# pigBond/olympics-mujoco

Hardware: AMD Instinct MI355X
Metric: env-steps/sec, 4096 UnitreeH1.walk envs per GPU, obs+reward+done+ctrl HIP kernel (higher is better)
Workload: dtype f64; 1 GPU; UnitreeH1.walk config-2: fused K1+K5 over one [T,N] block per step; T=400, envs_per_gpu=4096, launch_regime=[T,N] block per launch, io=qpos/qvel f64 + action f32 in; obs/reward/ctrl f32 + absorbing u8 out, parallelism=env-sharded x1, no data-path collective

## Files before the change

olympics-mujoco_amd/csrc/k1_il_step.hip:

```cpp
#include <cstdlib>

#include "oly_common.h"

namespace {

constexpr int THREADS = 256;
typedef unsigned int u32x4 __attribute__((ext_vector_type(4)));

template <int NQ, int NV, int NGRF, int NACT, int NU, int NOBS>
struct StaticDims {
  static constexpr int nq = NQ, nv = NV, n_grf = NGRF, n_act = NACT, nu = NU, n_obs = NOBS;
  static constexpr bool is_static = true;
  static constexpr int n_obs_ct = NOBS;
  template <int ROWS, int TH>
  static constexpr int max_chunks() {
    return (ROWS * (NQ + NV + NGRF) / 2 + ROWS * NACT / 4 + TH - 1) / TH;
  }
  __device__ explicit StaticDims(const IlDev*) {}
};
struct DynDims {
  int nq, nv, n_grf, n_act, nu, n_obs;
  static constexpr bool is_static = false;
  static constexpr int n_obs_ct = 1;
  template <int ROWS, int TH>
  static constexpr int max_chunks() { return 1; }
  __device__ explicit DynDims(const IlDev* m)
      : nq(m->nq), nv(m->nv), n_grf(m->n_grf), n_act(m->n_act), nu(m->nu), n_obs(m->n_obs) {}
};

struct IlArgs {
  const IlDev* md;
  long R;
  int N;
  const double* qpos;
  const double* qvel;
  const float* action;
  const double* grf;
  const double* prev_in;
  double* prev_out;
  void* obs;
  float* reward;
  uint8_t* absorbing;
  uint8_t* fall_code;
  void* ctrl;
  int fast;
  long tile0;
};

template <int ROWS, class D>
struct Carve {
  int q, v, g, a, tab_off, tab_str, tab_csrc, tab_act, total;
  __host__ __device__ Carve(int nq, int nv, int n_grf, int n_act, int nu, int n_obs) {
    auto al = [](int x) { return (x + 15) & ~15; };
    q = 0;
    v = q + ROWS * nq * 8;
    g = v + ROWS * nv * 8;
    a = al(g + ROWS * n_grf * 8);
    tab_off = al(a + ROWS * n_act * 4);
    tab_str = al(tab_off + n_obs * 4);
    tab_csrc = al(tab_str + n_obs * 4);
    tab_act = al(tab_csrc + nu * 4);
    total = al(tab_act + 4 * nu * 8);
  }
};

#ifndef OLY_K1_NT
#define OLY_K1_NT 1
#endif
typedef float f32x4 __attribute__((ext_vector_type(4)));
typedef double f64x2 __attribute__((ext_vector_type(2)));
__device__ __forceinline__ u32x4 ld16(const u32x4* p) {
  return (OLY_K1_NT & 1) ? __builtin_nontemporal_load(p) : *p;
}
__device__ __forceinline__ void st16(f32x4* p, f32x4 v) {
  if (OLY_K1_NT & 2) __builtin_nontemporal_store(v, p); else *p = v;
}
__device__ __forceinline__ void st16(f64x2* p, f64x2 v) {
  if (OLY_K1_NT & 2) __builtin_nontemporal_store(v, p); else *p = v;
}

#ifndef OLY_K1_ABLATE
#define OLY_K1_ABLATE 0
#endif

constexpr int FAST_FALL = 8;

template <int ROWS, class D, bool OBS64, bool CTRL64>
__global__ __launch_bounds__(THREADS) void il_step_kernel(IlArgs p) {
  extern __shared__ __attribute__((aligned(16))) unsigned char lds[];
  const IlDev* __restrict__ md = p.md;
  const D d(md);
  const Carve<ROWS, D> cv(d.nq, d.nv, d.n_grf, d.n_act, d.nu, d.n_obs);
  const int tid = threadIdx.x;
  const int lane = tid & 63;
  const long row0 = (p.tile0 + blockIdx.x) * ROWS;
  const int rows = (p.R - row0 < ROWS) ? (int)(p.R - row0) : ROWS;
  const bool full = (rows == ROWS) && p.fast;

  double* sq = reinterpret_cast<double*>(lds + cv.q);
  double* sv = reinterpret_cast<double*>(lds + cv.v);
  double* sg = reinterpret_cast<double*>(lds + cv.g);
  float* sa = reinterpret_cast<float*>(lds + cv.a);
  int* t_off = reinterpret_cast<int*>(lds + cv.tab_off);
  int* t_str = reinterpret_cast<int*>(lds + cv.tab_str);
  int* t_cidx = reinterpret_cast<int*>(lds + cv.tab_csrc);
  double* t_act = reinterpret_cast<double*>(lds + cv.tab_act);

  auto col_off = [&](int sidx) -> int {
    if (sidx < d.nq) return sidx;
    if (sidx < d.nq + d.nv) return ROWS * d.nq + (sidx - d.nq);
    return ROWS * (d.nq + d.nv) + (sidx - d.nq - d.nv);
  };
  auto col_str = [&](int sidx) -> int {
    if (sidx < d.nq) return d.nq;
    if (sidx < d.nq + d.nv) return d.nv;
    return d.n_grf;
  };
  const int first_grf = d.n_obs - d.n_grf;

  const int cq = ROWS * d.nq / 2, cvv = ROWS * d.nv / 2, cg = ROWS * d.n_grf / 2;
  const int ca = p.action ? ROWS * d.n_act / 4 : 0;
  const int cd = cq + cvv + cg;
  const int total = (OLY_K1_ABLATE & 2) ? 0 : cd + ca;
  u32x4* ld = reinterpret_cast<u32x4*>(sq);
  u32x4* la = reinterpret_cast<u32x4*>(sa);
  constexpr int MAXC = D::template max_chunks<ROWS, THREADS>();
  u32x4 regs[MAXC];
  const bool reg_staged = D::is_static && full;
  if (reg_staged) {
    const u32x4* gq = reinterpret_cast<const u32x4*>(p.qpos + row0 * d.nq);
    const u32x4* gv = reinterpret_cast<const u32x4*>(p.qvel + row0 * d.nv);
    const u32x4* gg = reinterpret_cast<const u32x4*>(p.grf ? p.grf + row0 * d.n_grf : nullptr);
    const u32x4* ga = reinterpret_cast<const u32x4*>(p.action ? p.action + row0 * d.n_act : nullptr);
#pragma unroll
    for (int k = 0; k < MAXC; ++k) {
      const int g = tid + k * THREADS;
      if (g < total) {
        const u32x4* src = g < cq ? gq + g : (g < cq + cvv ? gv + (g - cq) : (g < cd ? gg + (g - cq - cvv) : ga + (g - cd)));
        regs[k] = *src;
      }
    }
  }

  for (int i = tid; i < d.n_obs; i += THREADS) {
    const int sidx = md->src[i];
    t_off[i] = col_off(sidx);
    t_str[i] = col_str(sidx);
  }
  for (int j = tid; j < d.nu; j += THREADS) {
    const int k = md->ctrl_src[j];
    t_cidx[j] = k;
    const int kk = k < 0 ? 0 : k;
    t_act[j] = md->act_mean[kk];
    t_act[d.nu + j] = md->act_delta[kk];
    t_act[2 * d.nu + j] = md->ctrl_lo[kk];
    t_act[3 * d.nu + j] = md->ctrl_hi[kk];
  }
  constexpr int OW = OBS64 ? 2 : 4;
  const bool fixed_cols = D::is_static && ((THREADS * OW) % d.n_obs == 0);
  int my_off[OW], my_str[OW];
  if (fixed_cols) {
    const int c0 = (tid * OW) % d.n_obs;
#pragma unroll
    for (int k = 0; k < OW; ++k) {
      const int sidx = md->src[c0 + k];
      my_off[k] = col_off(sidx);
      my_str[k] = col_str(sidx);
    }
// ... 400 lines not shown
      const unsigned ab = (code != 0 && use_abs) ? 1u : 0u;
      if (rt == OLY_REWARD_NONE) {
        p.reward[gr] = 0.0f;
      } else {
        if (gr < p.N) p.reward[gr] = rew_f(p.prev_in[gr]);
        if (gr + p.N < p.R)
          p.reward[gr + p.N] = rew_f(x);
        else
          p.prev_out[gr - (p.R - p.N)] = x;
      }
      unsigned a4 = 0, c4 = 0;
#pragma unroll
      for (int k = 0; k < 4; ++k) {
        const int srcl = (lane & 15) * 4 + k;
        a4 |= (unsigned)__shfl((int)ab, srcl, 64) << (8 * k);
        c4 |= (unsigned)__shfl((int)code, srcl, 64) << (8 * k);
      }
      if (lane < 16) {
        const long q4 = (row0 + (r - lane)) / 4 + lane;
        reinterpret_cast<unsigned*>(p.absorbing)[q4] = a4;
        if (p.fall_code) reinterpret_cast<unsigned*>(p.fall_code)[q4] = c4;
      }
    }

    {
      double v[NIT][OW];
#pragma unroll
      for (int it = 0; it < NIT; ++it)
#pragma unroll
        for (int k = 0; k < OW; ++k) {
          v[it][k] = sq[e_off[it][k]];
          if (NG > 0 && ((e_grf >> (it * OW + k)) & 1u)) v[it][k] = v[it][k] / 1000.0;
        }
#pragma unroll
      for (int it = 0; it < NIT; ++it) {
        const int i = tid + it * THREADS;
        if (it * THREADS + THREADS <= NOV || i < NOV) {
          if (OBS64) {
            f64x2 o;
            o.x = v[it][0]; o.y = v[it][OW - 1];
            st16(reinterpret_cast<f64x2*>(static_cast<double*>(p.obs) + row0 * NO) + i, o);
          } else {
            f32x4 o;
            o.x = (float)v[it][0]; o.y = (float)v[it][1 % OW];
            o.z = (float)v[it][2 % OW]; o.w = (float)v[it][3 % OW];
            st16(reinterpret_cast<f32x4*>(static_cast<float*>(p.obs) + row0 * NO) + i, o);
          }
        }
      }
    }

    if (with_ctrl) {
#pragma unroll
      for (int it = 0; it < NCI; ++it) {
        const int i = tid + it * THREADS;
        if (it * THREADS + THREADS <= NCV || i < NCV) {
          double u[CW];
#pragma unroll
          for (int q = 0; q < CW; ++q) {
            const int ai = c_aidx[it][q], j = c_j[it][q];
            const double a = (double)sa[ai < 0 ? 0 : ai];
            double x = a * t_act[NU + j] + t_act[j];
            const double lo = t_act[2 * NU + j], hi = t_act[3 * NU + j];
            if (x < lo) x = lo;
            if (x > hi) x = hi;
            u[q] = ai < 0 ? 0.0 : x;
          }
          if (CTRL64) {
            f64x2 o;
            o.x = u[0]; o.y = u[CW - 1];
            st16(reinterpret_cast<f64x2*>(static_cast<double*>(p.ctrl) + row0 * NU) + i, o);
          } else {
            f32x4 o;
            o.x = (float)u[0]; o.y = (float)u[1 % CW]; o.z = (float)u[2 % CW]; o.w = (float)u[3 % CW];
            st16(reinterpret_cast<f32x4*>(static_cast<float*>(p.ctrl) + row0 * NU) + i, o);
          }
        }
      }
    }
    __syncthreads();
  }
}

template <bool CTRL64>
__global__ __launch_bounds__(THREADS) void il_ctrl_kernel(const IlDev* __restrict__ md, long total,
                                                          const float* __restrict__ action,
                                                          void* __restrict__ ctrl) {
  const int nu = md->nu, n_act = md->n_act;
  const long stride = (long)gridDim.x * THREADS;
  for (long e = (long)blockIdx.x * THREADS + threadIdx.x; e < total; e += stride) {
    const long r = e / nu;
    const int j = (int)(e - r * nu);
    const int k = md->ctrl_src[j];
    double u = 0.0;
    if (k >= 0) {
      u = (double)action[r * n_act + k] * md->act_delta[k] + md->act_mean[k];
      if (u < md->ctrl_lo[k]) u = md->ctrl_lo[k];
      if (u > md->ctrl_hi[k]) u = md->ctrl_hi[k];
    }
    if (CTRL64)
      static_cast<double*>(ctrl)[e] = u;
    else
      static_cast<float*>(ctrl)[e] = (float)u;
  }
}

constexpr int DYN_ROWS = 64;

struct DynCarve {
  int a, eo, co, tact, total;
  __host__ __device__ DynCarve(int nq, int nv, int n_grf, int n_act, int nu, int n_obs) {
    auto al = [](int x) { return (x + 15) & ~15; };
    a = al(DYN_ROWS * (nq + nv + n_grf) * 8);
    eo = al(a + DYN_ROWS * n_act * 4);
    co = al(eo + DYN_ROWS * n_obs * 4);
    tact = al(co + DYN_ROWS * nu * 4);
    total = al(tact + 4 * nu * 8);
  }
};

template <bool OBS64, bool CTRL64>
__global__ __launch_bounds__(THREADS) void il_dyn_tile_kernel(IlArgs p) {
  constexpr int ROWS = DYN_ROWS;
  extern __shared__ __attribute__((aligned(16))) unsigned char lds[];
  const IlDev* __restrict__ md = p.md;
  const int nq = md->nq, nv = md->nv, n_grf = md->n_grf, n_act = md->n_act, nu = md->nu, n_obs = md->n_obs;
  const DynCarve cv(nq, nv, n_grf, n_act, nu, n_obs);
  const int tid = threadIdx.x, lane = tid & 63;
  double* sq = reinterpret_cast<double*>(lds);
  float* sa = reinterpret_cast<float*>(lds + cv.a);
  unsigned* eo = reinterpret_cast<unsigned*>(lds + cv.eo);
  int* co = reinterpret_cast<int*>(lds + cv.co);
  double* t_act = reinterpret_cast<double*>(lds + cv.tact);
  const bool with_ctrl = p.ctrl != nullptr;
  const int first_grf = n_obs - n_grf;

  auto col_off = [&](int sidx) -> int {
    if (sidx < nq) return sidx;
    if (sidx < nq + nv) return ROWS * nq + (sidx - nq);
    return ROWS * (nq + nv) + (sidx - nq - nv);
  };
  auto col_str = [&](int sidx) -> int { return sidx < nq ? nq : (sidx < nq + nv ? nv : n_grf); };

  for (int e = tid; e < ROWS * n_obs; e += THREADS) {
    const int r = e / n_obs, c = e - r * n_obs;
    const int sidx = md->src[c];
    eo[e] = (unsigned)(col_off(sidx) + r * col_str(sidx)) | (c >= first_grf && n_grf > 0 ? 0x80000000u : 0u);
  }
  for (int e = tid; e < ROWS * nu; e += THREADS) {
    const int r = e / nu, j = e - r * nu;
    const int k = md->ctrl_src[j];
    co[e] = k < 0 ? -1 : (((r * n_act + k) << 8) | j);
  }
  for (int j = tid; j < nu; j += THREADS) {
    const int k = md->ctrl_src[j];
    const int kk = k < 0 ? 0 : k;
    t_act[j] = md->act_mean[kk];
    t_act[nu + j] = md->act_delta[kk];
    t_act[2 * nu + j] = md->ctrl_lo[kk];
    t_act[3 * nu + j] = md->ctrl_hi[kk];
  }
  const int nf = md->n_fall;
  const int rt = md->reward_type;
  const int rew_sidx = md->reward_sidx;
  const bool rew_grf = n_grf > 0 && md->reward_idx >= first_grf;
  const double tvel = md->target_velocity;
  const int use_abs = md->use_absorbing;
  auto rew_f = [&](double s) -> float {
    if (rt == OLY_REWARD_TARGET_VELOCITY) {
      const double dv = s - tvel;
      return (float)exp(-(dv * dv));
    }
    return (float)s;
  };

  const int cq = ROWS * nq / 2, cvv = ROWS * nv / 2, cg = ROWS * n_grf / 2;
  const int ca = with_ctrl ? ROWS * n_act / 4 : 0;
  constexpr int KQ = 5, KG = 1, KA = 3;
  u32x4 rq[KQ], rv[KQ], rg[KG], ra[KA];
  u32x4* lq = reinterpret_cast<u32x4*>(sq);
  u32x4* lv = lq + cq;
// ... 108 lines not shown
        }
        if (OBS64) {
          f64x2 o;
          o.x = v[0]; o.y = v[OW - 1];
          st16(reinterpret_cast<f64x2*>(static_cast<double*>(p.obs) + row0 * n_obs) + i, o);
        } else {
          f32x4 o;
          o.x = (float)v[0]; o.y = (float)v[1 % OW]; o.z = (float)v[2 % OW]; o.w = (float)v[3 % OW];
          st16(reinterpret_cast<f32x4*>(static_cast<float*>(p.obs) + row0 * n_obs) + i, o);
        }
      }
    }

    if (with_ctrl) {
      constexpr int CW = CTRL64 ? 2 : 4;
      const int ncv = ROWS * nu / CW;
      for (int i = tid; i < ncv; i += THREADS) {
        double u[CW];
#pragma unroll
        for (int q = 0; q < CW; ++q) {
          const int c = co[i * CW + q];
          const int j = c & 0xff, ai = c >> 8;
          const double a = (double)sa[c < 0 ? 0 : ai];
          double x = a * t_act[nu + (c < 0 ? 0 : j)] + t_act[c < 0 ? 0 : j];
          const double lo = t_act[2 * nu + (c < 0 ? 0 : j)], hi = t_act[3 * nu + (c < 0 ? 0 : j)];
          if (x < lo) x = lo;
          if (x > hi) x = hi;
          u[q] = c < 0 ? 0.0 : x;
        }
        if (CTRL64) {
          f64x2 o;
          o.x = u[0]; o.y = u[CW - 1];
          st16(reinterpret_cast<f64x2*>(static_cast<double*>(p.ctrl) + row0 * nu) + i, o);
        } else {
          f32x4 o;
          o.x = (float)u[0]; o.y = (float)u[1 % CW]; o.z = (float)u[2 % CW]; o.w = (float)u[3 % CW];
          st16(reinterpret_cast<f32x4*>(static_cast<float*>(p.ctrl) + row0 * nu) + i, o);
        }
      }
    }
    __syncthreads();
  }
}

using H1Dims = StaticDims<17, 17, 0, 11, 11, 32>;
using AtlasDims = StaticDims<16, 16, 0, 10, 10, 30>;
using TalosDims = StaticDims<18, 18, 0, 12, 12, 34>;
using H1FFDims = StaticDims<17, 17, 6, 11, 11, 38>;
using TalosFFDims = StaticDims<18, 18, 6, 12, 12, 40>;
using H1ArmsDims = StaticDims<25, 25, 0, 19, 19, 48>;
using H1ArmsNoBackDims = StaticDims<24, 24, 0, 18, 18, 46>;
using AtlasBackDims = StaticDims<19, 19, 0, 13, 13, 36>;
using ArmsNoBack28Dims = StaticDims<28, 28, 0, 22, 22, 54>;
using AtlasFullDims = StaticDims<31, 31, 0, 25, 25, 60>;
using TalosFullDims = StaticDims<30, 30, 0, 24, 24, 58>;

template <int ROWS, class D>
int launch_generic(oly_ctx* ctx, IlArgs a, long tile0, int out_flags, hipStream_t s) {
  const IlDev& h = ctx->il_host;
  Carve<ROWS, D> cv(h.nq, h.nv, h.n_grf, h.n_act, h.nu, h.n_obs);
  const long tiles = (a.R + ROWS - 1) / ROWS - tile0;
  if (tiles <= 0) return OLY_OK;
  if (tiles > 0x7fffffffL) OLY_FAIL(ctx, OLY_EINVAL, "oly_il_step: too many rows");
  a.tile0 = tile0;
  dim3 grid((unsigned)tiles), block(THREADS);
  const bool o64 = out_flags & OLY_OUT_OBS_F64, c64 = out_flags & OLY_OUT_CTRL_F64;
#define OLY_K1(O, C_)                                                                       \
  do {                                                                                      \
    auto k = il_step_kernel<ROWS, D, O, C_>;                                                \
    if (cv.total > 48 * 1024)                                                               \
      OLY_HIP(ctx, hipFuncSetAttribute(reinterpret_cast<const void*>(k),                    \
                                       hipFuncAttributeMaxDynamicSharedMemorySize, cv.total)); \
    hipLaunchKernelGGL(k, grid, block, cv.total, s, a);                                     \
  } while (0)
  if (o64 && c64) OLY_K1(true, true);
  else if (o64) OLY_K1(true, false);
  else if (c64) OLY_K1(false, true);
  else OLY_K1(false, false);
#undef OLY_K1
  OLY_LAUNCH_CHECK(ctx, "il_step_kernel");
  return OLY_OK;
}

template <int ROWS, class D>
int launch_fast(oly_ctx* ctx, IlArgs a, int out_flags, int wg_per_cu, hipStream_t s) {
  const long nfull = a.R / ROWS;
  if (nfull > 0) {
    const int lds = ROWS * (D::nq + D::nv + D::n_grf) * 8 + ROWS * D::n_act * 4 + 4 * D::nu * 8;
    int per_cu = (160 * 1024) / lds;
    if (per_cu > 8) per_cu = 8;
    if (wg_per_cu > 0) per_cu = wg_per_cu;
    long want = (long)ctx->num_cu * per_cu;
    if (want > nfull) want = nfull;
    IlArgs b = a;
    b.tile0 = nfull;
    dim3 grid((unsigned)want), block(THREADS);
    const bool o64 = out_flags & OLY_OUT_OBS_F64, c64 = out_flags & OLY_OUT_CTRL_F64;
#define OLY_K1T(O, C_)                                                                      \
  do {                                                                                      \
    auto k = il_tile_kernel<ROWS, D, O, C_>;                                                \
    if (lds > 48 * 1024)                                                                    \
      OLY_HIP(ctx, hipFuncSetAttribute(reinterpret_cast<const void*>(k),                    \
                                       hipFuncAttributeMaxDynamicSharedMemorySize, lds));   \
    hipLaunchKernelGGL(k, grid, block, lds, s, b);                                          \
  } while (0)
    if (o64 && c64) OLY_K1T(true, true);
    else if (o64) OLY_K1T(true, false);
    else if (c64) OLY_K1T(false, true);
    else OLY_K1T(false, false);
#undef OLY_K1T
    OLY_LAUNCH_CHECK(ctx, "il_tile_kernel");
  }
  if (nfull * ROWS < a.R) return launch_generic<ROWS, D>(ctx, a, nfull, out_flags, s);
  return OLY_OK;
}

int launch_dyn(oly_ctx* ctx, IlArgs a, int out_flags, hipStream_t s) {
  const IlDev& h = ctx->il_host;
  const DynCarve cv(h.nq, h.nv, h.n_grf, h.n_act, h.nu, h.n_obs);
  const long nfull = (a.fast && cv.total <= 150 * 1024) ? a.R / DYN_ROWS : 0;
  if (nfull > 0) {
    int per_cu = (160 * 1024) / cv.total;
    if (per_cu > 4) per_cu = 4;
    if (per_cu < 1) per_cu = 1;
    long want = (long)ctx->num_cu * per_cu;
    if (want > nfull) want = nfull;
    IlArgs b = a;
    b.tile0 = nfull;
    dim3 grid((unsigned)want), block(THREADS);
    const bool o64 = out_flags & OLY_OUT_OBS_F64, c64 = out_flags & OLY_OUT_CTRL_F64;
#define OLY_K1D(O, C_)                                                                      \
  do {                                                                                      \
    auto k = il_dyn_tile_kernel<O, C_>;                                                     \
    if (cv.total > 48 * 1024)                                                               \
      OLY_HIP(ctx, hipFuncSetAttribute(reinterpret_cast<const void*>(k),                    \
                                       hipFuncAttributeMaxDynamicSharedMemorySize, cv.total)); \
    hipLaunchKernelGGL(k, grid, block, cv.total, s, b);                                     \
  } while (0)
    if (o64 && c64) OLY_K1D(true, true);
    else if (o64) OLY_K1D(true, false);
    else if (c64) OLY_K1D(false, true);
    else OLY_K1D(false, false);
#undef OLY_K1D
    OLY_LAUNCH_CHECK(ctx, "il_dyn_tile_kernel");
  }
  if (nfull * DYN_ROWS < a.R) return launch_generic<DYN_ROWS, DynDims>(ctx, a, nfull, out_flags, s);
  return OLY_OK;
}

inline bool al16(const void* p) { return (reinterpret_cast<uintptr_t>(p) & 15) == 0; }

}

extern "C" int oly_il_configure(oly_ctx* ctx, const oly_il_model* m) {
  if (!ctx || !m) return OLY_EINVAL;
  const int n_spec = m->n_pos + m->n_vel;
  const int n_obs = n_spec - m->n_drop + m->n_grf;
  if (m->nq <= 0 || m->nv <= 0 || m->n_pos < 0 || m->n_vel < 0 || m->n_drop < 0 || m->n_grf < 0 ||
      m->n_drop > n_spec || n_obs <= 0 || n_obs > OLY_MAX_OBS || m->n_act < 0 ||
      m->n_act > OLY_MAX_ACT || m->nu < m->n_act || m->nu > OLY_MAX_ACT || m->n_fall < 0 ||
      m->n_fall > OLY_MAX_FALL)
    OLY_FAIL(ctx, OLY_EINVAL, "oly_il_configure: bad shape (n_obs=%d n_act=%d nu=%d n_fall=%d)",
             n_obs, m->n_act, m->nu, m->n_fall);
  if (!m->qpos_adr || !m->qvel_adr || (m->n_act && (!m->act_to_ctrl || !m->act_mean ||
      !m->act_delta || !m->ctrl_lo || !m->ctrl_hi)) || (m->n_fall && (!m->fall_idx || !m->fall_lo ||
      !m->fall_hi)))
    OLY_FAIL(ctx, OLY_EINVAL, "oly_il_configure: NULL table");
  ctx->il_ok = false;
  IlDev& h = ctx->il_host;
  memset(&h, 0, sizeof(h));
  h.nq = m->nq; h.nv = m->nv; h.n_pos = m->n_pos; h.n_vel = m->n_vel; h.n_drop = m->n_drop;
  h.n_grf = m->n_grf; h.n_act = m->n_act; h.nu = m->nu; h.n_obs = n_obs; h.n_fall = m->n_fall;
  h.reward_type = m->reward_type; h.reward_idx = m->reward_idx;
  h.use_absorbing = m->use_absorbing_states; h.target_velocity = m->target_velocity;
  if (h.reward_type < OLY_REWARD_NONE || h.reward_type > OLY_REWARD_X_POS)
    OLY_FAIL(ctx, OLY_EINVAL, "oly_il_configure: unknown reward_type %d", h.reward_type);
  if (h.reward_type != OLY_REWARD_NONE && (h.reward_idx < 0 || h.reward_idx >= n_obs))
    OLY_FAIL(ctx, OLY_ERANGE, "oly_il_configure: reward_idx %d outside [0,%d)", h.reward_idx, n_obs);
  for (int c = 0; c < n_obs; ++c) {
    const int slot = c + m->n_drop;
    int s;
    if (slot < m->n_pos) {
      s = m->qpos_adr[slot];
      if (s < 0 || s >= m->nq) OLY_FAIL(ctx, OLY_ERANGE, "qpos_adr[%d]=%d outside nq=%d", slot, s, m->nq);
    } else if (slot < n_spec) {
      s = m->qvel_adr[slot - m->n_pos];
      if (s < 0 || s >= m->nv) OLY_FAIL(ctx, OLY_ERANGE, "qvel_adr[%d]=%d outside nv=%d", slot - m->n_pos, s, m->nv);
      s += m->nq;
    } else {
      s = m->nq + m->nv + (slot - n_spec);
    }
    h.src[c] = (short)s;
  }
  for (int k = 0; k < m->n_fall; ++k) {
    if (m->fall_idx[k] < 0 || m->fall_idx[k] >= n_obs)
      OLY_FAIL(ctx, OLY_ERANGE, "fall_idx[%d]=%d outside [0,%d)", k, m->fall_idx[k], n_obs);
    h.fall_idx[k] = m->fall_idx[k]; h.fall_lo[k] = m->fall_lo[k]; h.fall_hi[k] = m->fall_hi[k];
    h.fall_sidx[k] = h.src[m->fall_idx[k]];
  }
  h.reward_sidx = (h.reward_type != OLY_REWARD_NONE) ? h.src[h.reward_idx] : 0;
  for (int j = 0; j < m->nu; ++j) h.ctrl_src[j] = -1;
  for (int k = 0; k < m->n_act; ++k) {
    const int j = m->act_to_ctrl[k];
    if (j < 0 || j >= m->nu) OLY_FAIL(ctx, OLY_ERANGE, "act_to_ctrl[%d]=%d outside nu=%d", k, j, m->nu);
    h.ctrl_src[j] = (short)k;
    h.act_mean[k] = m->act_mean[k]; h.act_delta[k] = m->act_delta[k];
    h.ctrl_lo[k] = m->ctrl_lo[k]; h.ctrl_hi[k] = m->ctrl_hi[k];
  }
  OLY_HIP(ctx, hipSetDevice(ctx->device));
  OLY_HIP(ctx, hipMemcpy(ctx->il_dev, &h, sizeof(h), hipMemcpyHostToDevice));
  ctx->il_ok = true;
  return OLY_OK;
}

extern "C" int oly_il_obs_dim(const oly_ctx* ctx) {
  if (!ctx || !ctx->il_ok) return OLY_ENOTCONF;
  return ctx->il_host.n_obs;
}

extern "C" int oly_il_step(oly_ctx* ctx, int T, int N, const double* qpos, const double* qvel,
                           const float* action, const double* grf_mean, const double* prev_in,
                           double* prev_out, void* obs, float* reward, uint8_t* absorbing,
                           uint8_t* fall_code, void* ctrl, int out_flags, oly_stream stream) {
  if (!ctx) return OLY_EINVAL;
  if (!ctx->il_ok) OLY_FAIL(ctx, OLY_ENOTCONF, "oly_il_step before oly_il_configure");
  const IlDev& h = ctx->il_host;
  if (T < 0 || N < 0) OLY_FAIL(ctx, OLY_EINVAL, "oly_il_step: negative T or N");
  if (T == 0 || N == 0) return OLY_OK;
  if (!qpos || !qvel || !obs || !reward || !absorbing)
    OLY_FAIL(ctx, OLY_EINVAL, "oly_il_step: NULL required pointer");
  if (h.reward_type != OLY_REWARD_NONE && (!prev_in || !prev_out))
    OLY_FAIL(ctx, OLY_EINVAL, "oly_il_step: prev_in/prev_out required by the reward");
  if (T > 1 && prev_in == prev_out && prev_in)
    OLY_FAIL(ctx, OLY_EINVAL, "oly_il_step: prev_in must not alias prev_out when T > 1");
  if (h.n_grf > 0 && !grf_mean) OLY_FAIL(ctx, OLY_EINVAL, "oly_il_step: grf_mean required (n_grf=%d)", h.n_grf);
  if (ctrl && !action) OLY_FAIL(ctx, OLY_EINVAL, "oly_il_step: ctrl requested without action");
  IlArgs a;
  a.md = ctx->il_dev; a.R = (long)T * N; a.N = N; a.qpos = qpos; a.qvel = qvel; a.action = action;
  a.grf = h.n_grf ? grf_mean : nullptr; a.prev_in = prev_in; a.prev_out = prev_out; a.obs = obs;
  a.reward = reward; a.absorbing = absorbing; a.fall_code = fall_code; a.ctrl = ctrl;
  a.fast = al16(qpos) && al16(qvel) && al16(action) && al16(grf_mean) && al16(obs) && al16(ctrl) &&
           ((reinterpret_cast<uintptr_t>(absorbing) & 3) == 0) &&
           ((reinterpret_cast<uintptr_t>(fall_code) & 3) == 0);
  a.tile0 = 0;
  auto shape = [&](int nq, int na, int no, int ng = 0) {
    return h.nq == nq && h.nv == nq && h.n_grf == ng && h.n_act == na && h.nu == na && h.n_obs == no &&
           h.n_pos == nq && h.n_vel == nq && h.n_drop == 2;
  };
  const bool fast_ok = a.fast && h.n_fall <= FAST_FALL;
  static const int wg_env = [] { const char* e = getenv("OLY_K1_WG_PER_CU"); return e ? atoi(e) : 0; }();
  static const int rows_env = [] { const char* e = getenv("OLY_K1_ROWS"); return e ? atoi(e) : 0; }();
#define OLY_K1_FAST(DIMS, DEFROWS)                                                              \
  do {                                                                                          \
    const int rows = rows_env ? rows_env : DEFROWS;                                             \
    if (rows == 64) return launch_fast<64, DIMS>(ctx, a, out_flags, wg_env, oly_s(stream));     \
    return launch_fast<128, DIMS>(ctx, a, out_flags, wg_env, oly_s(stream));                    \
  } while (0)
  if (fast_ok && shape(17, 11, 32)) OLY_K1_FAST(H1Dims, 128);
  if (fast_ok && shape(16, 10, 30)) OLY_K1_FAST(AtlasDims, 128);
  if (fast_ok && shape(18, 12, 34)) OLY_K1_FAST(TalosDims, 128);
  if (fast_ok && shape(17, 11, 38, 6)) OLY_K1_FAST(H1FFDims, 128);
  if (fast_ok && shape(18, 12, 40, 6)) OLY_K1_FAST(TalosFFDims, 128);
  if (fast_ok && shape(25, 19, 48)) OLY_K1_FAST(H1ArmsDims, 128);
  if (fast_ok && shape(24, 18, 46)) return launch_fast<128, H1ArmsNoBackDims>(ctx, a, out_flags, wg_env, oly_s(stream));
  if (fast_ok && shape(19, 13, 36)) return launch_fast<128, AtlasBackDims>(ctx, a, out_flags, wg_env, oly_s(stream));
  if (fast_ok && shape(28, 22, 54)) return launch_fast<128, ArmsNoBack28Dims>(ctx, a, out_flags, wg_env, oly_s(stream));
  if (fast_ok && shape(31, 25, 60)) return launch_fast<128, AtlasFullDims>(ctx, a, out_flags, wg_env, oly_s(stream));
  if (fast_ok && shape(30, 24, 58)) return launch_fast<128, TalosFullDims>(ctx, a, out_flags, wg_env, oly_s(stream));
#undef OLY_K1_FAST
  static const int dyn_env = [] { const char* e = getenv("OLY_K1_DYN_TILE"); return e ? atoi(e) : 1; }();
  if (dyn_env) return launch_dyn(ctx, a, out_flags, oly_s(stream));
  return launch_generic<64, DynDims>(ctx, a, 0, out_flags, oly_s(stream));
}

extern "C" int oly_il_ctrl(oly_ctx* ctx, int N, const float* action, void* ctrl, int out_flags,
                           oly_stream stream) {
  if (!ctx) return OLY_EINVAL;
  if (!ctx->il_ok) OLY_FAIL(ctx, OLY_ENOTCONF, "oly_il_ctrl before oly_il_configure");
  if (N < 0 || (N > 0 && (!action || !ctrl))) OLY_FAIL(ctx, OLY_EINVAL, "oly_il_ctrl: bad argument");
  if (N == 0) return OLY_OK;
  const long total = (long)N * ctx->il_host.nu;
  long nb = (total + THREADS - 1) / THREADS;
  if (nb > 4096) nb = 4096;
  if (out_flags & OLY_OUT_CTRL_F64)
    hipLaunchKernelGGL(il_ctrl_kernel<true>, dim3((unsigned)nb), dim3(THREADS), 0, oly_s(stream), ctx->il_dev,
                       total, action, ctrl);
  else
    hipLaunchKernelGGL(il_ctrl_kernel<false>, dim3((unsigned)nb), dim3(THREADS), 0, oly_s(stream), ctx->il_dev,
                       total, action, ctrl);
  OLY_LAUNCH_CHECK(ctx, "il_ctrl_kernel");
  return OLY_OK;
}
```

olympics-mujoco_amd/csrc/oly_common.h:

```cpp
#pragma once

#include <hip/hip_runtime.h>

#include <cstdint>
#include <cstdio>
#include <cstring>

#include "../../include/olympic_hip.h"


struct IlDev {
  int nq, nv, n_pos, n_vel, n_drop, n_grf, n_act, nu, n_obs, n_fall;
  int reward_type, reward_idx, use_absorbing, reward_sidx;
  double target_velocity;
  short src[OLY_MAX_OBS];
  int fall_idx[OLY_MAX_FALL], fall_sidx[OLY_MAX_FALL];
  double fall_lo[OLY_MAX_FALL], fall_hi[OLY_MAX_FALL];
  short ctrl_src[OLY_MAX_ACT];
  double act_mean[OLY_MAX_ACT], act_delta[OLY_MAX_ACT], ctrl_lo[OLY_MAX_ACT], ctrl_hi[OLY_MAX_ACT];
};

struct A3Dev {
  int nq, nv, nu, period, delay_frames, n_obs, pad0, pad1;
  double target_radius, mass, goal_height_ref, goal_speed_ref;
  double clock_lut[4 * OLY_MAX_PERIOD];
  double motor_offset[16], gear[16];
};

struct ContactDev {
  int ngeom, floor_body, rfoot_body, lfoot_body;
  int* geom_bodyid;
};

struct GrfDev {
  int ngeom, n_pairs;
  int pair_a[OLY_MAX_GRF_PAIRS], pair_b[OLY_MAX_GRF_PAIRS];
  int* geom_group;
};

struct TrajDev {
  int n_keys, n_traj, len, pad;
  double* rows;
};

#define OLY_STATS_MAX_BLOCKS 1024

struct oly_ctx {
  int device;
  char err[512];
  IlDev* il_dev;
  IlDev il_host;
  bool il_ok;
  A3Dev* a3_dev;
  A3Dev a3_host;
  bool a3_ok;
  ContactDev contact;
  bool contact_ok;
  TrajDev traj;
  bool traj_ok;
  GrfDev grf;
  bool grf_ok;
  int* grf_group_host;
  double* stats_ws;
  size_t stats_ws_bytes;
  bool mlp_attr_done = false;
  bool disc_attr_done = false;
  bool roll_attr_done = false;
  unsigned upd_attr_done = 0;
  unsigned scan_attr_done = 0;
  unsigned ilmlp_attr_done = 0;
  unsigned discfit_attr_done = 0;
  unsigned gail_attr_done = 0;
  int num_cu;
  unsigned ilact_attr_done = 0;
  unsigned bcfit_attr_done = 0;
  unsigned sgact_attr_done = 0;
  unsigned iqq_attr_done = 0;
};

#define OLY_FAIL(ctx, code, ...)                                \
  do {                                                          \
    if (ctx) snprintf((ctx)->err, sizeof((ctx)->err), __VA_ARGS__); \
    return (code);                                              \
  } while (0)

#define OLY_HIP(ctx, expr)                                                             \
  do {                                                                                 \
    hipError_t e__ = (expr);                                                           \
    if (e__ != hipSuccess)                                                             \
      OLY_FAIL(ctx, OLY_EHIP, "%s failed: %s (%s:%d)", #expr, hipGetErrorString(e__), \
               __FILE__, __LINE__);                                                    \
  } while (0)

#define OLY_LAUNCH_CHECK(ctx, what)                                                           \
  do {                                                                                        \
    hipError_t e__ = hipGetLastError();                                                       \
    if (e__ != hipSuccess)                                                                    \
      OLY_FAIL(ctx, OLY_EHIP, "launch of %s failed: %s", what, hipGetErrorString(e__));       \
  } while (0)

int oly_stats_finish(oly_ctx* ctx, int nblocks, int64_t n, double* stats3_out, oly_stream stream);
int oly_masked_col_stats(oly_ctx* ctx, long B, int Dx, int D, const float* x, const int32_t* mask, double* colstats,
                         int accumulate, double* copy_out, oly_stream stream);
// ... 11 lines not shown
```

Measured before the change: 12.98 billion env-steps/s.

## Add small-tile fused IL step kernel for low env counts

Adds il_small_kernel, a compile-time-dimension kernel that handles 16/32/64 rows per block. Each block loads qpos/qvel/grf/action into registers, stages them in static LDS, and emits obs, ctrl, reward and packed absorbing/fall-code bytes. Obs, fall and reward columns are precomputed into packed offset words, and ctrl parameters into a u_tab table. launch_fast routes to this path when R is below 128 rows per CU, which gives more, smaller blocks and better occupancy for moderate env counts than the persistent tile kernel. The ctrl kernel also switches to 32-bit indexing and vectorized table loads.

```diff
diff --git a/olympics-mujoco_amd/csrc/k1_il_step.hip b/olympics-mujoco_amd/csrc/k1_il_step.hip
--- a/olympics-mujoco_amd/csrc/k1_il_step.hip
+++ b/olympics-mujoco_amd/csrc/k1_il_step.hip
@@ -83,7 +83,7 @@
 #define OLY_K1_ABLATE 0
 #endif
 
-constexpr int FAST_FALL = 8;
+constexpr int FAST_FALL = OLY_IL_FAST_FALL;
 
 template <int ROWS, class D, bool OBS64, bool CTRL64>
 __global__ __launch_bounds__(THREADS) void il_step_kernel(IlArgs p) {
@@ -650,21 +650,313 @@
   }
 }
 
-template <bool CTRL64>
-__global__ __launch_bounds__(THREADS) void il_ctrl_kernel(const IlDev* __restrict__ md, long total,
+template <int H, class D>
+__global__ __launch_bounds__(4 * H) void il_small_kernel(IlArgs p, int obs64, int ctrl64) {
+  static_assert(D::is_static, "small-tile kernel needs compile-time dimensions");
+  static_assert(H == 16 || H == 32 || H == 64, "tile heights: row0 stays a multiple of 16, rows fit wave 0");
+  constexpr int TH = 4 * H;
+  constexpr int NQ = D::nq, NV = D::nv, NG = D::n_grf, NA = D::n_act, NU = D::nu, NO = D::n_obs;
+  constexpr int ND = NQ + NV + NG;
+  constexpr int CQ = H * NQ / 2, CV = H * NV / 2, CG = H * NG / 2, CA = H * NA / 4;
+  constexpr int KQ = (CQ + TH - 1) / TH, KV = (CV + TH - 1) / TH, KG = (CG + TH - 1) / TH,
+                KA = (CA + TH - 1) / TH;
+  constexpr int NOV = H * NO / 4, NIT = (NOV + TH - 1) / TH;
+  constexpr int NCV = H * NU / 4, NCI = (NCV + TH - 1) / TH;
+  static_assert(NIT * 4 <= 32, "grf bitmask holds 32 values per lane");
+
+  __shared__ __attribute__((aligned(16))) unsigned char lds[H * ND * 8 + H * NA * 4];
+  double* sq = reinterpret_cast<double*>(lds);
+  float* sa = reinterpret_cast<float*>(lds + H * ND * 8);
+  const IlDev* __restrict__ md = p.md;
+  const int tid = threadIdx.x, lane = tid & 63;
+  const bool with_ctrl = p.ctrl != nullptr;
+  const long row0 = (long)blockIdx.x * H;
+  const int rows = (p.R - row0 < H) ? (int)(p.R - row0) : H;
+
+  auto lds_off = [&](int w, int r) -> int {
+    const int arr = w >> 24;
+    return (arr == 0 ? 0 : arr == 1 ? H * NQ : H * (NQ + NV)) + (w & 0xfff) + r * ((w >> 12) & 0xfff);
+  };
+  auto is_grf = [&](int w) -> bool { return NG > 0 && (w >> 24) == 2; };
+
+  u32x4 rq[KQ], rv[KV], rg[KG > 0 ? KG : 1], ra[KA];
+  double prev0 = 0.0;
+  int ow[NIT][4];
+  int cs[NCI][4];
+  f64x2 ut[NCI][4][2];
+  const bool full = rows == H;
+  auto chunk = [&](int k, int n) -> int {
+    const int g = tid + k * TH;
+    return (k * TH + TH <= n || g < n) ? g : n - 1;
+  };
+  if (full) {
+    const u32x4* gq = reinterpret_cast<const u32x4*>(p.qpos + row0 * NQ);
+    const u32x4* gv = reinterpret_cast<const u32x4*>(p.qvel + row0 * NV);
+#pragma unroll
+    for (int k = 0; k < KQ; ++k) rq[k] = ld16(gq + chunk(k, CQ));
+#pragma unroll
+    for (int k = 0; k < KV; ++k) rv[k] = ld16(gv + chunk(k, CV));
+    if (NG > 0) {
+      const u32x4* gg = reinterpret_cast<const u32x4*>(p.grf + row0 * NG);
+#pragma unroll
+      for (int k = 0; k < KG; ++k) rg[k] = ld16(gg + chunk(k, CG));
+    }
+    if (with_ctrl) {
+      const u32x4* ga = reinterpret_cast<const u32x4*>(p.action + row0 * NA);
+#pragma unroll
+      for (int k = 0; k < KA; ++k) ra[k] = ld16(ga + chunk(k, CA));
+    }
+    if (tid < H && row0 + tid < p.N && p.prev_in) prev0 = p.prev_in[row0 + tid];
+#pragma unroll
+    for (int it = 0; it < NIT; ++it)
+#pragma unroll
+      for (int k = 0; k < 4; ++k) {
+        const int e = (tid + it * TH) * 4 + k;
+        ow[it][k] = md->obs_col[e % NO];
+      }
+    if (with_ctrl) {
+#pragma unroll
+      for (int it = 0; it < NCI; ++it)
+#pragma unroll
+        for (int q = 0; q < 4; ++q) {
+          const int e = (tid + it * TH) * 4 + q;
+          const int j = e % NU;
+          cs[it][q] = md->ctrl_src[j];
+          ut[it][q][0] = *reinterpret_cast<const f64x2*>(&md->u_tab[j][0]);
+          ut[it][q][1] = *reinterpret_cast<const f64x2*>(&md->u_tab[j][2]);
+        }
+    }
+  }
+  int f_col[FAST_FALL];
+  double f_lo[FAST_FALL], f_hi[FAST_FALL];
+#pragma unroll
+  for (int k = 0; k < FAST_FALL; ++k) {
+    f_col[k] = md->fall_col[k];
+    f_lo[k] = md->fall_lo8[k];
+    f_hi[k] = md->fall_hi8[k];
+  }
+  const int rt = md->reward_type, rew_col = md->reward_col, use_abs = md->use_absorbing;
+  const double tvel = md->target_velocity;
+  auto rew_f = [&](double s) -> float {
+    if (rt == OLY_REWARD_TARGET_VELOCITY) {
+      const double dv = s - tvel;
+      return (float)exp(-(dv * dv));
+    }
+    return (float)s;
+  };
+  auto row_phase = [&](int r, double prev, unsigned& code, unsigned& ab) {
+    const long gr = row0 + r;
+    double fv[FAST_FALL];
+#pragma unroll
+    for (int k = 0; k < FAST_FALL; ++k) {
+      fv[k] = sq[lds_off(f_col[k], r)];
+      if (is_grf(f_col[k])) fv[k] = fv[k] / 1000.0;
+    }
+    double x = sq[lds_off(rew_col, r)];
+    if (is_grf(rew_col)) x = x / 1000.0;
+    code = 0;
+#pragma unroll
+    for (int k = FAST_FALL - 1; k >= 0; --k)
+      if (fv[k] < f_lo[k] || fv[k] > f_hi[k]) code = (unsigned)(k + 1);
+    ab = (code != 0 && use_abs) ? 1u : 0u;
+    if (rt == OLY_REWARD_NONE) {
+      p.reward[gr] = 0.0f;
+    } else {
+      if (gr < p.N) p.reward[gr] = rew_f(prev);
+      if (gr + p.N < p.R)
+        p.reward[gr + p.N] = rew_f(x);
+      else
+        p.prev_out[gr - (p.R - p.N)] = x;
+    }
+  };
+
+  if (!full) {
+    for (int i = tid; i < rows * NQ; i += TH) sq[i] = p.qpos[row0 * NQ + i];
+    for (int i = tid; i < rows * NV; i += TH) sq[H * NQ + i] = p.qvel[row0 * NV + i];
+    if (NG > 0)
+      for (int i = tid; i < rows * NG; i += TH) sq[H * (NQ + NV) + i] = p.grf[row0 * NG + i];
+    if (with_ctrl)
+      for (int i = tid; i < rows * NA; i += TH) sa[i] = p.action[row0 * NA + i];
+    __syncthreads();
+    if (tid < rows) {
+      const long gr = row0 + tid;
+      unsigned code, ab;
+      row_phase(tid, (gr < p.N && p.prev_in) ? p.prev_in[gr] : 0.0, code, ab);
+      p.absorbing[gr] = (uint8_t)ab;
+      if (p.fall_code) p.fall_code[gr] = (uint8_t)code;
+    }
+    for (int e = tid; e < rows * NO; e += TH) {
+      const int r = e / NO, w = md->obs_col[e - r * NO];
+      double v = sq[lds_off(w, r)];
+      if (is_grf(w)) v = v / 1000.0;
+      if (obs64)
+        static_cast<double*>(p.obs)[row0 * NO + e] = v;
+      else
+        static_cast<float*>(p.obs)[row0 * NO + e] = (float)v;
+    }
+    if (with_ctrl)
+      for (int e = tid; e < rows * NU; e += TH) {
+        const int r = e / NU, j = e - r * NU, k = md->ctrl_src[j];
+        const double a = (double)sa[r * NA + (k < 0 ? 0 : k)];
+        double x = a * md->u_tab[j][1] + md->u_tab[j][0];
+        const double lo = md->u_tab[j][2], hi = md->u_tab[j][3];
+        if (x < lo) x = lo;
+        if (x > hi) x = hi;
+        const double u = k < 0 ? 0.0 : x;
+        if (ctrl64)
+          static_cast<double*>(p.ctrl)[row0 * NU + e] = u;
+        else
+          static_cast<float*>(p.ctrl)[row0 * NU + e] = (float)u;
+      }
+    return;
+  }
+
+  int e_off[NIT][4];
+  unsigned e_grf = 0;
+#pragma unroll
+  for (int it = 0; it < NIT; ++it)
+#pragma unroll
+    for (int k = 0; k < 4; ++k) {
+      const int e = (tid + it * TH) * 4 + k;
+      const bool in = (it * TH + TH) * 4 <= H * NO || e < H * NO;
+      e_off[it][k] = in ? lds_off(ow[it][k], e / NO) : 0;
+      if (in && is_grf(ow[it][k])) e_grf |= 1u << (it * 4 + k);
+    }
+  int c_aidx[NCI][4];
+  if (with_ctrl) {
+#pragma unroll
+    for (int it = 0; it < NCI; ++it)
+#pragma unroll
+      for (int q = 0; q < 4; ++q) {
+        const int e = (tid + it * TH) * 4 + q;
+        const bool in = (it * TH + TH) * 4 <= H * NU || e < H * NU;
+        c_aidx[it][q] = (!in || cs[it][q] < 0) ? -1 : (e / NU) * NA + cs[it][q];
+      }
+  }
+
+  {
+    u32x4* lq = reinterpret_cast<u32x4*>(sq) + tid;
+    u32x4* lv = reinterpret_cast<u32x4*>(sq + H * NQ) + tid;
+    u32x4* la = reinterpret_cast<u32x4*>(sa) + tid;
+#pragma unroll
+    for (int k = 0; k < KQ; ++k)
+      if (k * TH + TH <= CQ || tid + k * TH < CQ) lq[k * TH] = rq[k];
+#pragma unroll
+    for (int k = 0; k < KV; ++k)
+      if (k * TH + TH <= CV || tid + k * TH < CV) lv[k * TH] = rv[k];
+    if (NG > 0) {
+      u32x4* lg = reinterpret_cast<u32x4*>(sq + H * (NQ + NV)) + tid;
+#pragma unroll
+      for (int k = 0; k < KG; ++k)
+        if (k * TH + TH <= CG || tid + k * TH < CG) lg[k * TH] = rg[k];
+    }
+    if (with_ctrl) {
+#pragma unroll
+      for (int k = 0; k < KA; ++k)
+        if (k * TH + TH <= CA || tid + k * TH < CA) la[k * TH] = ra[k];
+    }
+  }
+  if (TH == 64) {
+    __builtin_amdgcn_fence(__ATOMIC_RELEASE, "wavefront");
+    __builtin_amdgcn_wave_barrier();
+    __builtin_amdgcn_fence(__ATOMIC_ACQUIRE, "wavefront");
+  } else {
+    __syncthreads();
+  }
+
+  {
+    double v[NIT][4];
+#pragma unroll
+    for (int it = 0; it < NIT; ++it)
+#pragma unroll
+      for (int k = 0; k < 4; ++k) {
+        v[it][k] = sq[e_off[it][k]];
+        if (NG > 0 && ((e_grf >> (it * 4 + k)) & 1u)) v[it][k] = v[it][k] / 1000.0;
+      }
+#pragma unroll
+    for (int it = 0; it < NIT; ++it) {
+      const int i = tid + it * TH;
+      if (it * TH + TH <= NOV || i < NOV) {
+        if (obs64) {
+          f64x2 a, b;
+          a.x = v[it][0]; a.y = v[it][1]; b.x = v[it][2]; b.y = v[it][3];
+          f64x2* o = reinterpret_cast<f64x2*>(static_cast<double*>(p.obs) + row0 * NO) + 2 * i;
+          st16(o, a);
+          st16(o + 1, b);
+        } else {
+          f32x4 o;
+          o.x = (float)v[it][0]; o.y = (float)v[it][1]; o.z = (float)v[it][2]; o.w = (float)v[it][3];
+          st16(reinterpret_cast<f32x4*>(static_cast<float*>(p.obs) + row0 * NO) + i, o);
+        }
+      }
+    }
+  }
+
+  if (with_ctrl) {
+#pragma unroll
+    for (int it = 0; it < NCI; ++it) {
+      const int i = tid + it * TH;
+      if (it * TH + TH <= NCV || i < NCV) {
+        double u[4];
+#pragma unroll
+        for (int q = 0; q < 4; ++q) {
+          const int ai = c_aidx[it][q];
+          const double a = (double)sa[ai < 0 ? 0 : ai];
+          double x = a * ut[it][q][0].y + ut[it][q][0].x;
+          const double lo = ut[it][q][1].x, hi = ut[it][q][1].y;
+          if (x < lo) x = lo;
+          if (x > hi) x = hi;
+          u[q] = ai < 0 ? 0.0 : x;
+        }
+        if (ctrl64) {
+          f64x2 a, b;
+          a.x = u[0]; a.y = u[1]; b.x = u[2]; b.y = u[3];
+          f64x2* o = reinterpret_cast<f64x2*>(static_cast<double*>(p.ctrl) + row0 * NU) + 2 * i;
+          st16(o, a);
+          st16(o + 1, b);
+        } else {
+          f32x4 o;
+          o.x = (float)u[0]; o.y = (float)u[1]; o.z = (float)u[2]; o.w = (float)u[3];
+          st16(reinterpret_cast<f32x4*>(static_cast<float*>(p.ctrl) + row0 * NU) + i, o);
+        }
+      }
+    }
+  }
+
+  if (tid < 64) {
+    unsigned code = 0, ab = 0;
+    if (tid < H) row_phase(tid, prev0, code, ab);
+    unsigned a4 = 0, c4 = 0;
+#pragma unroll
+    for (int k = 0; k < 4; ++k) {
+      const int srcl = (lane & 15) * 4 + k;
+      a4 |= (unsigned)__shfl((int)ab, srcl, 64) << (8 * k);
+      c4 |= (unsigned)__shfl((int)code, srcl, 64) << (8 * k);
+    }
+    if (lane < H / 4) {
+      const long q4 = row0 / 4 + lane;
+      reinterpret_cast<unsigned*>(p.absorbing)[q4] = a4;
+      if (p.fall_code) reinterpret_cast<unsigned*>(p.fall_code)[q4] = c4;
+    }
+  }
+}
+
+template <bool CTRL64, class I>
+__global__ __launch_bounds__(THREADS) void il_ctrl_kernel(const IlDev* __restrict__ md, I total, I nu, I n_act,
                                                           const float* __restrict__ action,
                                                           void* __restrict__ ctrl) {
-  const int nu = md->nu, n_act = md->n_act;
-  const long stride = (long)gridDim.x * THREADS;
-  for (long e = (long)blockIdx.x * THREADS + threadIdx.x; e < total; e += stride) {
-    const long r = e / nu;
+  const I stride = (I)gridDim.x * THREADS;
+  for (I e = (I)blockIdx.x * THREADS + threadIdx.x; e < total; e += stride) {
+    const I r = e / nu;
     const int j = (int)(e - r * nu);
     const int k = md->ctrl_src[j];
+    const f64x2 md_ = *reinterpret_cast<const f64x2*>(&md->u_tab[j][0]);
+    const f64x2 lh = *reinterpret_cast<const f64x2*>(&md->u_tab[j][2]);
     double u = 0.0;
     if (k >= 0) {
-      u = (double)action[r * n_act + k] * md->act_delta[k] + md->act_mean[k];
-      if (u < md->ctrl_lo[k]) u = md->ctrl_lo[k];
-      if (u > md->ctrl_hi[k]) u = md->ctrl_hi[k];
+      u = (double)action[r * n_act + (I)k] * md_.y + md_.x;
+      if (u < lh.x) u = lh.x;
+      if (u > lh.y) u = lh.y;
     }
     if (CTRL64)
       static_cast<double*>(ctrl)[e] = u;
@@ -939,8 +1231,28 @@
   return OLY_OK;
 }
 
+template <class D>
+int launch_step(oly_ctx* ctx, const IlArgs& a, long cu, int out_flags, hipStream_t s) {
+  const int o64 = (out_flags & OLY_OUT_OBS_F64) ? 1 : 0, c64 = (out_flags & OLY_OUT_CTRL_F64) ? 1 : 0;
+  if (a.R < 32 * cu)
+    hipLaunchKernelGGL((il_small_kernel<16, D>), dim3((unsigned)((a.R + 15) / 16)), dim3(64), 0, s, a, o64, c64);
+  else if (a.R < 64 * cu)
+    hipLaunchKernelGGL((il_small_kernel<32, D>), dim3((unsigned)((a.R + 31) / 32)), dim3(128), 0, s, a, o64, c64);
+  else
+    hipLaunchKernelGGL((il_small_kernel<64, D>), dim3((unsigned)((a.R + 63) / 64)), dim3(256), 0, s, a, o64, c64);
+  OLY_LAUNCH_CHECK(ctx, "il_small_kernel");
+  return OLY_OK;
+}
+
+bool step_enabled() {
+  static const int v = [] { const char* e = getenv("OLY_K1_STEP"); return e ? atoi(e) : 1; }();
+  return v != 0;
+}
+
 template <int ROWS, class D>
 int launch_fast(oly_ctx* ctx, IlArgs a, int out_flags, int wg_per_cu, hipStream_t s) {
+  const long cu = ctx->num_cu > 0 ? ctx->num_cu : 256;
+  if (step_enabled() && a.R < 128 * cu) return launch_step<D>(ctx, a, cu, out_flags, s);
   const long nfull = a.R / ROWS;
   if (nfull > 0) {
     const int lds = ROWS * (D::nq + D::nv + D::n_grf) * 8 + ROWS * D::n_act * 4 + 4 * D::nu * 8;
@@ -1064,6 +1376,25 @@
     h.act_mean[k] = m->act_mean[k]; h.act_delta[k] = m->act_delta[k];
     h.ctrl_lo[k] = m->ctrl_lo[k]; h.ctrl_hi[k] = m->ctrl_hi[k];
   }
+  auto col_word = [&](int sidx) -> int {
+    if (sidx < h.nq) return OLY_IL_COL(sidx, h.nq, 0);
+    if (sidx < h.nq + h.nv) return OLY_IL_COL(sidx - h.nq, h.nv, 1);
+    return OLY_IL_COL(sidx - h.nq - h.nv, h.n_grf, 2);
+  };
+  for (int c = 0; c < n_obs; ++c) h.obs_col[c] = col_word(h.src[c]);
+  for (int k = 0; k < OLY_IL_FAST_FALL; ++k) {
+    const bool used = k < h.n_fall;
+    h.fall_col[k] = col_word(used ? h.fall_sidx[k] : 0);
+    h.fall_lo8[k] = used ? h.fall_lo[k] : -__builtin_huge_val();
+    h.fall_hi8[k] = used ? h.fall_hi[k] : __builtin_huge_val();
+  }
+  h.reward_col = col_word(h.reward_sidx);
+  for (int j = 0; j < m->nu; ++j) {
+    const int k = h.ctrl_src[j];
+    if (k < 0) continue;
+    h.u_tab[j][0] = h.act_mean[k]; h.u_tab[j][1] = h.act_delta[k];
+    h.u_tab[j][2] = h.ctrl_lo[k]; h.u_tab[j][3] = h.ctrl_hi[k];
+  }
   OLY_HIP(ctx, hipSetDevice(ctx->device));
   OLY_HIP(ctx, hipMemcpy(ctx->il_dev, &h, sizeof(h), hipMemcpyHostToDevice));
   ctx->il_ok = true;
@@ -1136,15 +1467,26 @@
   if (!ctx->il_ok) OLY_FAIL(ctx, OLY_ENOTCONF, "oly_il_ctrl before oly_il_configure");
   if (N < 0 || (N > 0 && (!action || !ctrl))) OLY_FAIL(ctx, OLY_EINVAL, "oly_il_ctrl: bad argument");
   if (N == 0) return OLY_OK;
-  const long total = (long)N * ctx->il_host.nu;
+  const long nu = ctx->il_host.nu, n_act = ctx->il_host.n_act;
+  const long total = (long)N * nu;
   long nb = (total + THREADS - 1) / THREADS;
   if (nb > 4096) nb = 4096;
-  if (out_flags & OLY_OUT_CTRL_F64)
-    hipLaunchKernelGGL(il_ctrl_kernel<true>, dim3((unsigned)nb), dim3(THREADS), 0, oly_s(stream), ctx->il_dev,
-                       total, action, ctrl);
-  else
-    hipLaunchKernelGGL(il_ctrl_kernel<false>, dim3((unsigned)nb), dim3(THREADS), 0, oly_s(stream), ctx->il_dev,
-                       total, action, ctrl);
+  const bool c64 = out_flags & OLY_OUT_CTRL_F64;
+  if (total < (1L << 31)) {
+    typedef unsigned U;
+    if (c64)
+      hipLaunchKernelGGL((il_ctrl_kernel<true, U>), dim3((unsigned)nb), dim3(THREADS), 0, oly_s(stream), ctx->il_dev,
+                         (U)total, (U)nu, (U)n_act, action, ctrl);
+    else
+      hipLaunchKernelGGL((il_ctrl_kernel<false, U>), dim3((unsigned)nb), dim3(THREADS), 0, oly_s(stream), ctx->il_dev,
+                         (U)total, (U)nu, (U)n_act, action, ctrl);
+  } else if (c64) {
+    hipLaunchKernelGGL((il_ctrl_kernel<true, long>), dim3((unsigned)nb), dim3(THREADS), 0, oly_s(stream), ctx->il_dev,
+                       total, nu, n_act, action, ctrl);
+  } else {
+    hipLaunchKernelGGL((il_ctrl_kernel<false, long>), dim3((unsigned)nb), dim3(THREADS), 0, oly_s(stream), ctx->il_dev,
+                       total, nu, n_act, action, ctrl);
+  }
   OLY_LAUNCH_CHECK(ctx, "il_ctrl_kernel");
   return OLY_OK;
 }
diff --git a/olympics-mujoco_amd/csrc/oly_common.h b/olympics-mujoco_amd/csrc/oly_common.h
--- a/olympics-mujoco_amd/csrc/oly_common.h
+++ b/olympics-mujoco_amd/csrc/oly_common.h
@@ -9,6 +9,8 @@
 #include "../../include/olympic_hip.h"
 
 
+#define OLY_IL_FAST_FALL 8
+
 struct IlDev {
   int nq, nv, n_pos, n_vel, n_drop, n_grf, n_act, nu, n_obs, n_fall;
   int reward_type, reward_idx, use_absorbing, reward_sidx;
@@ -18,7 +20,13 @@
   double fall_lo[OLY_MAX_FALL], fall_hi[OLY_MAX_FALL];
   short ctrl_src[OLY_MAX_ACT];
   double act_mean[OLY_MAX_ACT], act_delta[OLY_MAX_ACT], ctrl_lo[OLY_MAX_ACT], ctrl_hi[OLY_MAX_ACT];
+  int obs_col[OLY_MAX_OBS];
+  int fall_col[OLY_IL_FAST_FALL];
+  double fall_lo8[OLY_IL_FAST_FALL], fall_hi8[OLY_IL_FAST_FALL];
+  int reward_col;
+  alignas(16) double u_tab[OLY_MAX_ACT][4];
 };
+#define OLY_IL_COL(local, stride, array) ((local) | ((stride) << 12) | ((array) << 24))
 
 struct A3Dev {
   int nq, nv, nu, period, delay_frames, n_obs, pad0, pad1;
```

Measured after the change: 12.99 billion env-steps/s (median of 4 runs). No clear change (+0.1%).
